# cs4247/music-transcription

Hardware: AMD Instinct MI355X
Metric: 30 s audio chunks/sec (mel+CNNRNN forward) (higher is better)
Workload: dtype f16; 1 GPU; CNNRNNModel inference, batch=32x30 s synthetic 16 kHz audio, mel+CNN-RNN HIP path (BASELINE.json configs[1]); batch_per_gpu=32, frames=938, coscheduled_batches_per_forward=4, streams_per_gpu=4, batches_in_flight=16, parallelism=dp1 (independent chunks)

## Files before the change

### music-transcription_amd/csrc/lstm.hip

```cpp
#include "lstm_handoff.h"
#include <stdlib.h>

namespace mt {

struct LstmArgs {
    const float* gx;
    const float* w_hh;
    float* hx;
    unsigned* status;
    int B, T, H;
    int g0;
    int ngl;
    float* gates_out;
    float* cx;
    const float* w_ihx;
    const float* bias;
    const float* hx_prev;
    int sleep_first, sleep_retry;
};

__device__ __forceinline__ float sigmoidf_(float x) { return __builtin_amdgcn_rcpf(1.0f + __expf(-x)); }
__device__ __forceinline__ float tanhf_(float x) { return fmaf(2.0f, __builtin_amdgcn_rcpf(1.0f + __expf(-2.0f * x)), -1.0f); }
constexpr unsigned H_POISON = 0xFFFFFFFFu;
constexpr int PAYLOAD_POLL_SLEEP = 10;
constexpr int PAYLOAD_POLL_SLEEP_BUSY = 18;
constexpr int PAYLOAD_POLL_SLEEP_TRAIN = 12;

#ifdef MT_LSTM_DIAG
__device__ unsigned long long mt_lstm_diag[1024][8];
#define DIAG_STAMP(i) do { if (tid == 0) { const long long n_ = __builtin_amdgcn_s_memrealtime(); dg[i] += n_ - tl; tl = n_; } } while (0)
#else
#define DIAG_STAMP(i) do { } while (0)
#endif

typedef __attribute__((__vector_size__(4 * sizeof(int)))) int i32x4_t;
__device__ __forceinline__ i32x4_t raw_rsrc(const void* p, unsigned bytes) {
    const unsigned long long a = (unsigned long long)p;
    i32x4_t r;
    r[0] = __builtin_amdgcn_readfirstlane((int)(unsigned)a);
    r[1] = __builtin_amdgcn_readfirstlane((int)((unsigned)(a >> 32) & 0xffffu));
    r[2] = __builtin_amdgcn_readfirstlane((int)bytes);
    r[3] = 0x00020000;
    return r;
}
__device__ __forceinline__ void asm_load_b128_sc1(u32x4& dst, int voff, i32x4_t rsrc) {
    asm volatile("buffer_load_dwordx4 %0, %1, %2, 0 offen sc1" : "=v"(dst) : "v"(voff), "s"(rsrc));
}
template <int N> __device__ __forceinline__ void vm_wait() { asm volatile("s_waitcnt vmcnt(%0)" :: "n"(N)); }
__device__ __forceinline__ void vm_settle(u32x4& v) { asm volatile("" : "+v"(v)); }

template <int NKSW, bool TRAIN = false, bool XP = false, int NG = 1, bool G16 = false>
__global__ __launch_bounds__(XP ? 256 : 320, XP ? 1 : (NKSW > 8 ? 2 : 4)) void lstm_rec_kernel(LstmArgs a) {
    __shared__ __attribute__((aligned(16))) float red[4][64][20];
    __shared__ __attribute__((aligned(16))) f16_t hs[32][8];
    constexpr int GX_RING = XP ? 1 : 6;
    constexpr int GX_DMA = G16 ? 2 : 4;
    __shared__ __attribute__((aligned(16))) float gring[GX_RING][XP ? 4 : (G16 ? 512 : 1024)];
    __shared__ int abort_s;
    const int tid = threadIdx.x, wv = tid >> 6, lane = tid & 63;
    const int H = a.H, T = a.T, nkb = H >> 3, nks = H >> 4;
    const int kb = blockIdx.x, d = blockIdx.y, gbase = blockIdx.z * NG + a.g0;
    const int ngh = min(NG, a.g0 + a.ngl - gbase);
    const int b = lane & 31, hh = lane >> 5;

    if (!XP && wv == 4) {
        typedef __attribute__((address_space(1))) void gvoid_t;
        typedef __attribute__((address_space(3))) void lvoid_t;
        const size_t gd_blocks_l = (size_t)T * 2 * nkb;
        const int nslots = T * ngh;
        int is = 0, ig = 0;
        auto request = [&](int n) {
            const int tn = d ? (T - 1 - is) : is;
            const size_t blk = (size_t)(gbase + ig) * gd_blocks_l + ((size_t)tn * 2 + d) * nkb + kb;
            const char* src = (const char*)a.gx + blk * (G16 ? 2048 : 4096) + lane * 16;
            char* dst = (char*)&gring[n % GX_RING][0];
#pragma unroll
            for (int qq = 0; qq < GX_DMA; ++qq) __builtin_amdgcn_global_load_lds((gvoid_t*)(src + qq * 1024), (lvoid_t*)(dst + qq * 1024), 16, 0, 0);
            if (++ig == ngh) { ig = 0; ++is; }
        };
        for (int n = 0; n < GX_RING - 1 && n < nslots; ++n) request(n);
        if (GX_RING - 1 <= nslots) asm volatile("s_waitcnt vmcnt(%0)" :: "n"(GX_DMA * (GX_RING - 2)) : "memory");
        else asm volatile("s_waitcnt vmcnt(0)" ::: "memory");
        __builtin_amdgcn_s_barrier();
        for (int n = 0; n < nslots; ++n) {
            if (n + GX_RING - 1 < nslots) {
                request(n + GX_RING - 1);
                asm volatile("s_waitcnt vmcnt(%0)" :: "n"(GX_DMA * (GX_RING - 2)) : "memory");
            } else {
                asm volatile("s_waitcnt vmcnt(0)" ::: "memory");
            }
            __builtin_amdgcn_s_barrier();
            int ab;
            asm volatile("ds_read_b32 %0, %1\n\ts_waitcnt lgkmcnt(0)" : "=v"(ab) : "v"((unsigned)(size_t)(lvoid_t*)&abort_s) : "memory");
            if (ab) return;
            __builtin_amdgcn_s_barrier();
        }
        return;
    }

    const int r = lane & 31, q = r >> 3, rh = (r >> 2) & 1, p = r & 3;
    const int wrow = p * H + kb * 8 + 2 * q + rh;
    const float* wsrc = a.w_hh + ((size_t)d * 4 * H + wrow) * H;
    f16x8 w16[NKSW];
#pragma unroll
    for (int i = 0; i < NKSW; ++i) {
        const int ks = wv * NKSW + i, ksc = min(ks, nks - 1);
        const f32x4 w0 = *(const f32x4*)(wsrc + ksc * 16 + 8 * hh), w1 = *(const f32x4*)(wsrc + ksc * 16 + 8 * hh + 4);
#pragma unroll
        for (int j = 0; j < 4; ++j) {
            w16[i][j] = (ks < nks) ? (f16_t)w0[j] : (f16_t)0.0f;
            w16[i][4 + j] = (ks < nks) ? (f16_t)w1[j] : (f16_t)0.0f;
        }
    }

    constexpr int NKSX = XP ? 2 * NKSW : 1;
    f16x8 wx[NKSX];
    if (XP) {
        const float* wxsrc = a.w_ihx + ((size_t)d * 4 * H + wrow) * (2 * H);
#pragma unroll
        for (int i = 0; i < NKSX; ++i) {
            const int kx = wv * NKSX + i, kxc = min(kx, 2 * nks - 1);
            const f32x4 w0 = *(const f32x4*)(wxsrc + kxc * 16 + 8 * hh), w1 = *(const f32x4*)(wxsrc + kxc * 16 + 8 * hh + 4);
#pragma unroll
            for (int j = 0; j < 4; ++j) {
                wx[i][j] = (kx < 2 * nks) ? (f16_t)w0[j] : (f16_t)0.0f;
                wx[i][4 + j] = (kx < 2 * nks) ? (f16_t)w1[j] : (f16_t)0.0f;
            }
        }
    }

    const int jl = 2 * wv + hh;
    float cst[NG];
#pragma unroll
    for (int gi = 0; gi < NG; ++gi) cst[gi] = 0.0f;
    float bias4[4] = {0.0f, 0.0f, 0.0f, 0.0f};
    if (XP) {
#pragma unroll
        for (int pp = 0; pp < 4; ++pp) bias4[pp] = a.bias[(size_t)d * 4 * H + pp * H + kb * 8 + jl];
    }
    const size_t gd_blocks = (size_t)T * 2 * nkb;
    if (tid == 0) abort_s = 0;
    __syncthreads();
#ifdef MT_LSTM_DIAG
    unsigned long long dg[8] = {0, 0, 0, 0, 0, 0, 0, 0};
    long long tl = __builtin_amdgcn_s_memrealtime();
#endif

    u32x4 hq[NKSW];
    const bool pf = NG > 1 && ngh > 1;
    int ring = 0;
    for (int s = 0; s < T; ++s) {
        const int t = d ? (T - 1 - s) : s;
        const int tprev = d ? (t + 1) : (t - 1);
#pragma unroll
      for (int gi = 0; gi < NG; ++gi) {
        if (gi >= ngh) continue;
        const int g = gbase + gi;
        const int Bg = min(32, a.B - g * 32);
        float& c = cst[gi];
        char* hx_g = (char*)a.hx + (size_t)g * gd_blocks * 512;
        const __amdgpu_buffer_rsrc_t hrsrc = __builtin_amdgcn_make_buffer_rsrc(hx_g, 0, (int)(gd_blocks * 512), 0x00020000);
        const __amdgpu_buffer_rsrc_t xrsrc = __builtin_amdgcn_make_buffer_rsrc(
            XP ? (void*)((const char*)a.hx_prev + (size_t)g * gd_blocks * 512) : (void*)hx_g, 0, (int)(gd_blocks * 512), 0x00020000);

        u32x4 xr[NKSX];
        if (XP) {
#pragma unroll
            for (int i = 0; i < NKSX; ++i) {
                const int kx = wv * NKSX + i, dsel = kx >= nks ? 1 : 0, ksx = kx - dsel * nks;
                xr[i] = __builtin_amdgcn_raw_buffer_load_b128(xrsrc, (kx < 2 * nks) ? ((t * 2 + dsel) * nkb) * 512 + ksx * 1024 + lane * 16 : OOB_OFF, 0, 0);
            }
        }
        float gxv[4];
        if (XP) {
#pragma unroll
            for (int pp = 0; pp < 4; ++pp) gxv[pp] = bias4[pp];
        } else if (G16) {
            unsigned short raw[4];
#pragma unroll
            for (int pp = 0; pp < 4; ++pp) raw[pp] = ((const unsigned short*)gring[ring])[pp * 256 + jl * 32 + b];
            __builtin_amdgcn_sched_barrier(0);
#pragma unroll
            for (int pp = 0; pp < 4; ++pp) gxv[pp] = (float)__builtin_bit_cast(f16_t, raw[pp]);
        } else {
#pragma unroll
            for (int pp = 0; pp < 4; ++pp) gxv[pp] = gring[ring][pp * 256 + jl * 32 + b];
        }
        ring = ring + 1 == GX_RING ? 0 : ring + 1;
        f32x16 acc, accx;
#pragma unroll
        for (int e = 0; e < 16; ++e) acc[e] = accx[e] = 0.0f;
        if (XP && s == 0) {
#pragma unroll
            for (int i = 0; i < NKSX; ++i) accx = __builtin_amdgcn_mfma_f32_32x32x16_f16(wx[i], __builtin_bit_cast(f16x8, xr[i]), accx, 0, 0, 0);
            acc = accx;
        }
        if (s > 0) {
            {
                if (NG == 1) sleep64(a.sleep_first);
            }
            const int hbase = ((tprev * 2 + d) * nkb) * 512 + lane * 16;
            long long t1 = 0;
            const i32x4_t hr = raw_rsrc(hx_g, (unsigned)(gd_blocks * 512));
            for (unsigned it = 0;; ++it) {
                if (!pf || it > 0) {
#pragma unroll
                    for (int i = 0; i < NKSW; ++i) {
                        const int ks = wv * NKSW + i;
                        if (NG > 1) asm_load_b128_sc1(hq[i], (ks < nks) ? hbase + ks * 1024 : OOB_OFF, hr);
                        else hq[i] = __builtin_amdgcn_raw_buffer_load_b128(hrsrc, (ks < nks) ? hbase + ks * 1024 : OOB_OFF, 0, 16 );
                    }
                }
                if (NG > 1) {
                    static_assert(NG == 1 || (!TRAIN && !XP), "NG > 1 is the plain inference kernel: the hand-counted vmcnt does not cover TRAIN / XP stores and loads");
                    if (pf && it == 0 && wv == 0) vm_wait<1>();
                    else vm_wait<0>();
#pragma unroll
                    for (int i = 0; i < NKSW; ++i) vm_settle(hq[i]);
                }
                if (XP) {
                    if (it == 0) {
                        __builtin_amdgcn_sched_barrier(0);
#pragma unroll
                        for (int i = 0; i < NKSX; ++i) accx = __builtin_amdgcn_mfma_f32_32x32x16_f16(wx[i], __builtin_bit_cast(f16x8, xr[i]), accx, 0, 0, 0);
                        __builtin_amdgcn_sched_barrier(0);
                    }
                    acc = accx;
                }
                unsigned worst = 0;
#pragma unroll
                for (int i = 0; i < NKSW; ++i) {
                    worst = max(max(worst, max(hq[i][0], hq[i][1])), max(hq[i][2], hq[i][3]));
                    acc = __builtin_amdgcn_mfma_f32_32x32x16_f16(w16[i], __builtin_bit_cast(f16x8, hq[i]), acc, 0, 0, 0);
                }
                if (!__any(worst == H_POISON)) break;
#ifdef MT_LSTM_DIAG
                if (tid == 0) dg[7] += 1;
#endif
#pragma unroll
                for (int e = 0; e < 16; ++e) acc[e] = 0.0f;
                sleep64(a.sleep_retry);
                if ((it & 63u) == 63u && __hip_atomic_load(a.status, __ATOMIC_RELAXED, __HIP_MEMORY_SCOPE_AGENT) != 0) {
                    if (lane == 0) abort_s = 1;
                    break;
                }
                if ((it & 255u) == 255u) {
                    const long long now = __builtin_amdgcn_s_memrealtime();
                    if (t1 == 0) t1 = now;
                    else if (now - t1 > LSTM_SPIN_LIMIT_TICKS) {
                        if (lane == 0) {
                            __hip_atomic_store(a.status, 0x40000000u + (unsigned)s, __ATOMIC_RELAXED, __HIP_MEMORY_SCOPE_AGENT);
                            abort_s = 1;
                        }
                        break;
                    }
                }
            }
        }
        const bool wrap = gi + 1 >= ngh;
        const int sn = s + (wrap ? 1 : 0), gn = wrap ? gbase : g + 1;
        if (pf) {
            if (sn > 0 && sn < T) {
                const int tpn = d ? (T - sn) : (sn - 1);
                const i32x4_t nr = raw_rsrc((char*)a.hx + (size_t)gn * gd_blocks * 512, (unsigned)(gd_blocks * 512));
                const int nbase = ((tpn * 2 + d) * nkb) * 512 + lane * 16;
#pragma unroll
                for (int i = 0; i < NKSW; ++i) {
                    const int ks = wv * NKSW + i;
                    asm_load_b128_sc1(hq[i], (ks < nks) ? nbase + ks * 1024 : OOB_OFF, nr);
                }
            }
        }
#ifdef MT_LSTM_DIAG
        asm volatile("" :: "v"(acc[0]));
#endif
        DIAG_STAMP(2);
#pragma unroll
        for (int e4 = 0; e4 < 4; ++e4)
            *(f32x4*)(&red[wv][lane][4 * e4]) = f32x4{acc[4 * e4], acc[4 * e4 + 1], acc[4 * e4 + 2], acc[4 * e4 + 3]};
        __syncthreads();
        DIAG_STAMP(3);
        if (abort_s) {
            if (NG > 1) vm_wait<0>();
            return;
        }
        float pre[4];
        {
            const f32x4 r0 = *(const f32x4*)(&red[0][lane][4 * wv]), r1 = *(const f32x4*)(&red[1][lane][4 * wv]);
            const f32x4 r2 = *(const f32x4*)(&red[2][lane][4 * wv]), r3 = *(const f32x4*)(&red[3][lane][4 * wv]);
#pragma unroll
            for (int pp = 0; pp < 4; ++pp)
                pre[pp] = ((r0[pp] + r1[pp]) + (r2[pp] + r3[pp])) + ((XP || b < Bg) ? gxv[pp] : 0.0f);
        }
        const float ig = sigmoidf_(pre[0]), fg = sigmoidf_(pre[1]), gg = tanhf_(pre[2]), og = sigmoidf_(pre[3]);
        c = fmaf(fg, c, ig * gg);
        const float hval = og * tanhf_(c);
        if (TRAIN && b < Bg) {
            float* go = a.gates_out + (size_t)g * gd_blocks * 1024 + (((size_t)t * 2 + d) * nkb + kb) * 1024 + jl * 32 + b;
            go[0] = ig; go[256] = fg; go[512] = gg; go[768] = og;
            a.cx[(size_t)g * gd_blocks * 256 + (((size_t)t * 2 + d) * nkb + kb) * 256 + jl * 32 + b] = c;
        }
#ifdef MT_LSTM_DIAG
        asm volatile("" :: "v"(hval));
#endif
        DIAG_STAMP(4);
        hs[b][jl] = (f16_t)hval;
        DIAG_STAMP(5);
        __syncthreads();
        if (wv == 0) {
            const u32x4 piece = *(const u32x4*)(&hs[b][0]);
            const int hoff = ((t * 2 + d) * nkb) * 512 + (kb >> 1) * 1024 + ((kb & 1) * 32 + b) * 16;
            __builtin_amdgcn_raw_buffer_store_b128(piece, hrsrc, lane < 32 ? hoff : OOB_OFF, 0, 16 );
        }
        DIAG_STAMP(6);
      }
    }
    if (NG > 1) vm_wait<0>();
#ifdef MT_LSTM_DIAG
    if (tid == 0) {
        const int wg = (blockIdx.z * gridDim.y + blockIdx.y) * gridDim.x + blockIdx.x;
        for (int i = 0; i < 8; ++i) mt_lstm_diag[wg & 1023][i] = dg[i];
    }
#endif
}

template <int NK, bool TRAIN, bool G16>
__global__ __launch_bounds__(320, 4) void lstm_rec16_kernel(LstmArgs a) {
    __shared__ __attribute__((aligned(16))) float red[4][2][64][4];
    __shared__ __attribute__((aligned(16))) f16_t hs[32][8];
    constexpr int GX_RING = 6;
    constexpr int GX_DMA = G16 ? 2 : 4;
    __shared__ __attribute__((aligned(16))) float gring[GX_RING][G16 ? 512 : 1024];
    __shared__ int abort_s;
    const int tid = threadIdx.x, wv = tid >> 6, lane = tid & 63;
    const int H = a.H, T = a.T, nkb = H >> 3, nks = H >> 4;
    const int kb = blockIdx.x, d = blockIdx.y, g = blockIdx.z + a.g0;
    const int Bg = min(16, a.B - g * 32);
    const size_t gd_blocks = (size_t)T * 2 * nkb;

    if (wv == 4) {
        typedef __attribute__((address_space(1))) void gvoid_t;
        typedef __attribute__((address_space(3))) void lvoid_t;
        int is = 0;
        auto request = [&](int n) {
            const int tn = d ? (T - 1 - is) : is;
            const size_t blk = (size_t)g * gd_blocks + ((size_t)tn * 2 + d) * nkb + kb;
            const char* src = (const char*)a.gx + blk * (G16 ? 2048 : 4096) + lane * 16;
            char* dst = (char*)&gring[n % GX_RING][0];
#pragma unroll
            for (int qq = 0; qq < GX_DMA; ++qq) __builtin_amdgcn_global_load_lds((gvoid_t*)(src + qq * 1024), (lvoid_t*)(dst + qq * 1024), 16, 0, 0);
            ++is;
        };
        for (int n = 0; n < GX_RING - 1 && n < T; ++n) request(n);
        if (GX_RING - 1 <= T) asm volatile("s_waitcnt vmcnt(%0)" :: "n"(GX_DMA * (GX_RING - 2)) : "memory");
        else asm volatile("s_waitcnt vmcnt(0)" ::: "memory");
        __builtin_amdgcn_s_barrier();
        for (int n = 0; n < T; ++n) {
            if (n + GX_RING - 1 < T) {
                request(n + GX_RING - 1);
                asm volatile("s_waitcnt vmcnt(%0)" :: "n"(GX_DMA * (GX_RING - 2)) : "memory");
            } else {
                asm volatile("s_waitcnt vmcnt(0)" ::: "memory");
            }
            __builtin_amdgcn_s_barrier();
            int ab;
            asm volatile("ds_read_b32 %0, %1\n\ts_waitcnt lgkmcnt(0)" : "=v"(ab) : "v"((unsigned)(size_t)(lvoid_t*)&abort_s) : "memory");
            if (ab) return;
            __builtin_amdgcn_s_barrier();
        }
        return;
    }

    const int rr = lane & 15, kg = lane >> 4;
    f16x8 w16[2][NK];
#pragma unroll
    for (int mt = 0; mt < 2; ++mt) {
        const int wrow = (rr & 3) * H + kb * 8 + 4 * mt + (rr >> 2);
        const float* wsrc = a.w_hh + ((size_t)d * 4 * H + wrow) * H;
#pragma unroll
        for (int i = 0; i < NK; ++i) {
            const int k0 = (wv * NK + i) * 32 + 8 * kg, k0c = min(k0, H - 8);
            const f32x4 w0 = *(const f32x4*)(wsrc + k0c), w1 = *(const f32x4*)(wsrc + k0c + 4);
#pragma unroll
            for (int j = 0; j < 4; ++j) {
                w16[mt][i][j] = (k0 < H) ? (f16_t)w0[j] : (f16_t)0.0f;
                w16[mt][i][4 + j] = (k0 < H) ? (f16_t)w1[j] : (f16_t)0.0f;
            }
        }
    }
    const int n = lane & 15, rg = lane >> 4, jl = 4 * (wv & 1) + rg;
    const bool owner = wv < 2;
    float c = 0.0f;
    char* hx_g = (char*)a.hx + (size_t)g * gd_blocks * 512;
    const __amdgpu_buffer_rsrc_t hrsrc = __builtin_amdgcn_make_buffer_rsrc(hx_g, 0, (int)(gd_blocks * 512), 0x00020000);
    const __amdgpu_buffer_rsrc_t gors = __builtin_amdgcn_make_buffer_rsrc(TRAIN ? (void*)(a.gates_out + (size_t)g * gd_blocks * 1024) : (void*)a.hx, 0,
                                                                          (int)(gd_blocks * 4096), 0x00020000);
    const __amdgpu_buffer_rsrc_t cxrs = __builtin_amdgcn_make_buffer_rsrc(TRAIN ? (void*)(a.cx + (size_t)g * gd_blocks * 256) : (void*)a.hx, 0,
                                                                          (int)(gd_blocks * 1024), 0x00020000);
    const int vo_t = (n < Bg) ? (jl * 32 + n) * 4 : 0x7FFFF000;
    if (tid == 0) abort_s = 0;
    if (tid < 128) ((unsigned*)&hs[0][0])[tid] = 0u;
    __syncthreads();

    int ring = 0;
    for (int s = 0; s < T; ++s) {
        const int t = d ? (T - 1 - s) : s;
        const int tprev = d ? (t + 1) : (t - 1);
        float gxv[4];
        if (G16) {
            unsigned short raw[4];
#pragma unroll
            for (int pp = 0; pp < 4; ++pp) raw[pp] = ((const unsigned short*)gring[ring])[pp * 256 + jl * 32 + n];
            __builtin_amdgcn_sched_barrier(0);
#pragma unroll
            for (int pp = 0; pp < 4; ++pp) gxv[pp] = (float)__builtin_bit_cast(f16_t, raw[pp]);
        } else {
#pragma unroll
            for (int pp = 0; pp < 4; ++pp) gxv[pp] = gring[ring][pp * 256 + jl * 32 + n];
        }
        ring = ring + 1 == GX_RING ? 0 : ring + 1;
        f32x4 acc[2] = {{0.0f, 0.0f, 0.0f, 0.0f}, {0.0f, 0.0f, 0.0f, 0.0f}};
        if (s > 0) {
            sleep64(a.sleep_first);
            const int hbase = ((tprev * 2 + d) * nkb) * 512 + ((kg & 1) * 32 + n) * 16 + (kg >> 1) * 1024;
            long long t1 = 0;
            for (unsigned it = 0;; ++it) {
                u32x4 hq[NK];
#pragma unroll
                for (int i = 0; i < NK; ++i) {
                    const int ks = 2 * (wv * NK + i) + (kg >> 1);
                    hq[i] = __builtin_amdgcn_raw_buffer_load_b128(hrsrc, (ks < nks) ? hbase + (wv * NK + i) * 2048 : OOB_OFF, 0, 16 );
                }
                unsigned worst = 0;
#pragma unroll
                for (int i = 0; i < NK; ++i) {
                    worst = max(max(worst, max(hq[i][0], hq[i][1])), max(hq[i][2], hq[i][3]));
                    acc[0] = __builtin_amdgcn_mfma_f32_16x16x32_f16(w16[0][i], __builtin_bit_cast(f16x8, hq[i]), acc[0], 0, 0, 0);
                    acc[1] = __builtin_amdgcn_mfma_f32_16x16x32_f16(w16[1][i], __builtin_bit_cast(f16x8, hq[i]), acc[1], 0, 0, 0);
                }
                if (!__any(worst == H_POISON)) break;
                acc[0] = f32x4{0.0f, 0.0f, 0.0f, 0.0f}; acc[1] = f32x4{0.0f, 0.0f, 0.0f, 0.0f};
                sleep64(a.sleep_retry);
                if ((it & 63u) == 63u && __hip_atomic_load(a.status, __ATOMIC_RELAXED, __HIP_MEMORY_SCOPE_AGENT) != 0) {
                    if (lane == 0) abort_s = 1;
                    break;
                }
                if ((it & 255u) == 255u) {
                    const long long now = __builtin_amdgcn_s_memrealtime();
                    if (t1 == 0) t1 = now;
                    else if (now - t1 > LSTM_SPIN_LIMIT_TICKS) {
                        if (lane == 0) {
                            __hip_atomic_store(a.status, 0x40000000u + (unsigned)s, __ATOMIC_RELAXED, __HIP_MEMORY_SCOPE_AGENT);
                            abort_s = 1;
                        }
                        break;
                    }
                }
            }
        }
        *(f32x4*)(&red[wv][0][lane][0]) = acc[0];
        *(f32x4*)(&red[wv][1][lane][0]) = acc[1];
        __syncthreads();
        if (abort_s) return;
        float gate[4] = {0.0f, 0.0f, 0.0f, 0.0f};
        if (owner) {
            const int mt = wv;
            const f32x4 r0 = *(const f32x4*)(&red[0][mt][lane][0]), r1 = *(const f32x4*)(&red[1][mt][lane][0]);
            const f32x4 r2 = *(const f32x4*)(&red[2][mt][lane][0]), r3 = *(const f32x4*)(&red[3][mt][lane][0]);
            float pre[4];
#pragma unroll
            for (int pp = 0; pp < 4; ++pp) pre[pp] = ((r0[pp] + r1[pp]) + (r2[pp] + r3[pp])) + (n < Bg ? gxv[pp] : 0.0f);
            gate[0] = sigmoidf_(pre[0]); gate[1] = sigmoidf_(pre[1]); gate[2] = tanhf_(pre[2]); gate[3] = sigmoidf_(pre[3]);
            c = fmaf(gate[1], c, gate[0] * gate[2]);
            hs[n][jl] = (f16_t)(gate[3] * tanhf_(c));
        }
        __syncthreads();
        if (wv == 0) {
            const u32x4 piece = *(const u32x4*)(&hs[lane & 31][0]);
            const int hoff = ((t * 2 + d) * nkb) * 512 + (kb >> 1) * 1024 + ((kb & 1) * 32 + (lane & 31)) * 16;
            __builtin_amdgcn_raw_buffer_store_b128(piece, hrsrc, lane < 32 ? hoff : OOB_OFF, 0, 16 );
        }
        if (TRAIN && owner) {
            const int so = __builtin_amdgcn_readfirstlane((t * 2 + d) * nkb + kb);
#pragma unroll
            for (int pp = 0; pp < 4; ++pp) __builtin_amdgcn_raw_buffer_store_b32(__builtin_bit_cast(unsigned, gate[pp]), gors, vo_t + pp * 1024, so * 4096, 0);
            __builtin_amdgcn_raw_buffer_store_b32(__builtin_bit_cast(unsigned, c), cxrs, vo_t, so * 1024, 0);
        }
    }
}

template <int DT>
__global__ void lstm_relayout_kernel(const f16_t* __restrict__ hx, bf16_t* __restrict__ X, int ldx, float* __restrict__ Y, int ldy,
                                     int col_off, int B, int T, int H, int Hv, Div3 dv, unsigned mB, unsigned sB) {
    const int nkb = H >> 3, nkv = (Hv + 7) >> 3;
    const unsigned total = (unsigned)T * B * 2 * nkv;
    for (unsigned id = blockIdx.x * blockDim.x + threadIdx.x; id < total; id += gridDim.x * blockDim.x) {
        int kb, d, mi;
        div3(id, dv, kb, d, mi);
        const size_t m = (size_t)mi;
        const int t = (int)fast_div((unsigned)mi, (unsigned)B, mB, sB), b = mi - t * B, g = b >> 5, bl = b & 31;
        const f16_t* src = hx + ((((size_t)g * T + t) * 2 + d) * nkb) * 256 + (size_t)(kb >> 1) * 512 + ((kb & 1) * 32 + bl) * 8;
        const int c0 = col_off + d * Hv + kb * 8;
        const f16x8 h8 = *(const f16x8*)src;
        if (X) {
            if (DT == MT_DT_F16 && (c0 & 7) == 0 && kb * 8 + 8 <= Hv) {
                *(f16x8*)(X + m * ldx + c0) = h8;
            } else if ((c0 & 7) == 0 && kb * 8 + 8 <= Hv) {
                *(uint4*)(X + m * ldx + c0) = make_uint4(pack_bf16x2((float)h8[0], (float)h8[1]), pack_bf16x2((float)h8[2], (float)h8[3]),
                                                         pack_bf16x2((float)h8[4], (float)h8[5]), pack_bf16x2((float)h8[6], (float)h8[7]));
            } else {
                for (int j = 0; j < 8 && kb * 8 + j < Hv; ++j) X[m * ldx + c0 + j] = f32_to_h16<DT>((float)h8[j]);
            }
        }
        if (Y)
            for (int j = 0; j < 8 && kb * 8 + j < Hv; ++j) Y[m * ldy + c0 + j] = (float)h8[j];
    }
}

__global__ void lstm_unpack_kernel(const f16_t* __restrict__ hx, float* __restrict__ y, int B, int T, int H) {
    const int nkb = H >> 3;
    const size_t total = (size_t)T * B * 2 * H;
    for (size_t id = (size_t)blockIdx.x * blockDim.x + threadIdx.x; id < total; id += (size_t)gridDim.x * blockDim.x) {
        const int k = id % H;
        const int d = (id / H) & 1;
        const size_t bt = id / (2 * H);
        const int t = bt % T, b = bt / T, g = b >> 5, bl = b & 31;
        const f16_t* blk = hx + ((((size_t)g * T + t) * 2 + d) * nkb) * 256 + (size_t)(k >> 4) * 512;
        y[id] = (float)blk[(((k >> 3) & 1) * 32 + bl) * 8 + (k & 7)];
    }
}

template <int NKSW, bool G16>
static int launch_rec_plain(const LstmArgs& a, int ngroups, hipStream_t st) {
    const dim3 one_set(a.H >> 3, 2, 1);
    if constexpr (NKSW <= 8) {
        if (ngroups == 2) return persistent_launch(lstm_rec_kernel<NKSW, false, false, 2, G16>, one_set, 320, a, st, "mt_lstm_bidir_fwd");
        if (ngroups == 3) return persistent_launch(lstm_rec_kernel<NKSW, false, false, 3, G16>, one_set, 320, a, st, "mt_lstm_bidir_fwd");
        if (ngroups > 3) return persistent_launch(lstm_rec_kernel<NKSW, false, false, 4, G16>, dim3(a.H >> 3, 2, cdiv(ngroups, 4)), 320, a, st, "mt_lstm_bidir_fwd");
    }
    return persistent_launch(lstm_rec_kernel<NKSW, false, false, 1, G16>, dim3(a.H >> 3, 2, ngroups), 320, a, st, "mt_lstm_bidir_fwd");
}

template <int NKSW>
static int launch_rec(const LstmArgs& a, int ngroups, bool g16, hipStream_t st) {
    const dim3 per_group(a.H >> 3, 2, ngroups);
    if constexpr (NKSW <= 8) {
        static const bool c16 = !(getenv("MT_LSTM_C16") && atoi(getenv("MT_LSTM_C16")) == 0);
        constexpr int NK16 = (NKSW + 1) / 2;
        if (c16 && !a.w_ihx && a.B <= 16 && ngroups == 1) {
            if (a.cx) return persistent_launch(lstm_rec16_kernel<NK16, true, false>, per_group, 320, a, st, "mt_lstm_bidir_fwd_train");
            if (g16) return persistent_launch(lstm_rec16_kernel<NK16, false, true>, per_group, 320, a, st, "mt_lstm_bidir_fwd");
            return persistent_launch(lstm_rec16_kernel<NK16, false, false>, per_group, 320, a, st, "mt_lstm_bidir_fwd");
        }
        if (a.w_ihx) return persistent_launch(lstm_rec_kernel<NKSW, false, true>, per_group, 256, a, st, "mt_lstm_bidir_fwd_xproj");
    }
    if (a.cx) return persistent_launch(lstm_rec_kernel<NKSW, true, false>, per_group, 320, a, st, "mt_lstm_bidir_fwd_train");
    return g16 ? launch_rec_plain<NKSW, true>(a, ngroups, st) : launch_rec_plain<NKSW, false>(a, ngroups, st);
}

}

using namespace mt;

extern "C" size_t mt_lstm_gx_bytes(int B, int T, int H) { return (size_t)cdiv(B, 32) * T * 2 * (H >> 3) * 4096; }
extern "C" size_t mt_lstm_hx_bytes(int B, int T, int H) { return (size_t)cdiv(B, 32) * T * 2 * (H >> 3) * 512; }
extern "C" size_t mt_lstm_sync_bytes(int B, int H) { (void)B; (void)H; return 512; }

static int lstm_fwd_impl(const float* gx, const float* w_hh, float* hx, void* sync_ws, size_t sync_bytes,
                         int B, int T, int H, int flags, mt_stream_t stream, float* cx = nullptr,
                         const float* w_ihx = nullptr, const float* bias = nullptr, const float* hx_prev = nullptr) {
    MT_REQUIRE((gx || w_ihx) && w_hh && hx && sync_ws, MT_EINVAL, "mt_lstm_bidir_fwd: null pointer");
    MT_REQUIRE(B > 0 && T > 0 && H >= 16 && H % 16 == 0 && H <= 1024, MT_EUNSUPPORTED,
               "mt_lstm_bidir_fwd: hidden size %d unsupported (multiple of 16, <= 1024)", H);
    MT_REQUIRE(sync_bytes >= mt_lstm_sync_bytes(B, H), MT_EWORKSPACE, "mt_lstm_bidir_fwd: sync workspace too small");
    const int nkb = H >> 3, ng = cdiv(B, 32);
    const bool g16 = (flags & MT_GX_F16) != 0;
    MT_REQUIRE(!g16 || (!cx && !w_ihx), MT_EINVAL, "mt_lstm_bidir_fwd_ex: MT_GX_F16 is for plain inference launches only");
    MT_REQUIRE((size_t)T * 2 * nkb * 512 < ((size_t)1 << 31), MT_EUNSUPPORTED, "mt_lstm_bidir_fwd: T*H too large for one buffer descriptor");
    MT_REQUIRE(!cx || (size_t)T * 2 * nkb * 4096 < ((size_t)1 << 31), MT_EUNSUPPORTED, "mt_lstm_bidir_fwd_train: T*H too large for one buffer descriptor of the gates");
    MT_REQUIRE((((size_t)w_hh | (size_t)w_ihx) & 15) == 0, MT_EINVAL, "mt_lstm_bidir_fwd: weight matrices must be 16-byte aligned");
    hipStream_t st = (hipStream_t)stream;
    MT_CHECK_HIP(hipMemsetAsync(sync_ws, 0, mt_lstm_sync_bytes(B, H), st));
    MT_CHECK_HIP(hipMemsetAsync(hx, 0xFF, mt_lstm_hx_bytes(B, T, H), st));
    static const int env_first = getenv("MT_LSTM_POLL_FIRST") ? atoi(getenv("MT_LSTM_POLL_FIRST")) : -1;
    static const int env_retry = getenv("MT_LSTM_POLL_RETRY") ? atoi(getenv("MT_LSTM_POLL_RETRY")) : -1;
    LstmArgs a{gx, w_hh, hx, (unsigned*)sync_ws, B, T, H, 0, 0,
               cx ? const_cast<float*>(gx) : nullptr, cx, w_ihx, bias, hx_prev,
               env_first >= 0 ? env_first : (cx ? PAYLOAD_POLL_SLEEP_TRAIN : ((!w_ihx && mt_persistent_cus_in_flight(stream) > 0) ? PAYLOAD_POLL_SLEEP_BUSY : PAYLOAD_POLL_SLEEP)),
               env_retry >= 0 ? env_retry : 0};
    const int zmax = (256 / (2 * nkb)) > 0 ? (256 / (2 * nkb)) : 1;
    const int nksw = cdiv(nkb / 2, 4);
    const int per_launch = (cx || w_ihx || nksw > 8) ? zmax : 4 * zmax;
    for (int g0 = 0; g0 < ng; g0 += per_launch) {
        a.g0 = g0;
        const int n = (ng - g0) < per_launch ? (ng - g0) : per_launch;
        a.ngl = n;
        int rc;
        if (nksw <= 1) rc = launch_rec<1>(a, n, g16, st);
        else if (nksw <= 2) rc = launch_rec<2>(a, n, g16, st);
        else if (nksw <= 4) rc = launch_rec<4>(a, n, g16, st);
        else if (nksw <= 8) rc = launch_rec<8>(a, n, g16, st);
        else rc = launch_rec<16>(a, n, g16, st);
        if (rc != MT_OK) return rc;
    }
    return MT_OK;
}

extern "C" int mt_lstm_bidir_fwd(const float* gx, const float* w_hh, float* hx, void* sync_ws, size_t sync_bytes,
                                 int B, int T, int H, mt_stream_t stream) {
    return lstm_fwd_impl(gx, w_hh, hx, sync_ws, sync_bytes, B, T, H, 0, stream);
}

extern "C" int mt_lstm_bidir_fwd_xproj(const float* hx_prev, const float* w_ihx, const float* bias, const float* w_hh, float* hx,
                                       void* sync_ws, size_t sync_bytes, int B, int T, int H, mt_stream_t stream) {
    MT_REQUIRE(hx_prev && w_ihx && bias && hx_prev != hx, MT_EINVAL, "mt_lstm_bidir_fwd_xproj: bad arguments");
    MT_REQUIRE(H <= 512, MT_EUNSUPPORTED, "mt_lstm_bidir_fwd_xproj: H=%d > 512 (the W_ih slice lives in registers)", H);
    return lstm_fwd_impl(nullptr, w_hh, hx, sync_ws, sync_bytes, B, T, H, 0, stream, nullptr, w_ihx, bias, hx_prev);
}

extern "C" int mt_lstm_bidir_fwd_train(float* gx_inout, const float* w_hh, float* hx, float* cx, void* sync_ws, size_t sync_bytes,
                                       int B, int T, int H, mt_stream_t stream) {
    MT_REQUIRE(cx, MT_EINVAL, "mt_lstm_bidir_fwd_train: null cx");
    return lstm_fwd_impl(gx_inout, w_hh, hx, sync_ws, sync_bytes, B, T, H, 0, stream, cx);
}

extern "C" int mt_lstm_bidir_fwd_ex(const float* gx, const float* w_hh, float* hx, void* sync_ws, size_t sync_bytes,
                                    int B, int T, int H, int flags, mt_stream_t stream) {
    MT_REQUIRE(flags == 0 || flags == MT_GX_F16, MT_EINVAL, "mt_lstm_bidir_fwd_ex: flags must be 0 or MT_GX_F16 (gx is f16)");
    return lstm_fwd_impl(gx, w_hh, hx, sync_ws, sync_bytes, B, T, H, flags, stream);
}

extern "C" int mt_lstm_relayout_dt(const float* hx, void* X, int ldx, float* Y, int ldy, int col_off, int B, int T, int H, int Hv,
                                   int dt, mt_stream_t stream) {
    MT_REQUIRE(hx && (X || Y) && H % 16 == 0 && Hv > 0 && Hv <= H && col_off >= 0, MT_EINVAL, "mt_lstm_relayout_ex: bad arguments");
    MT_REQUIRE((!X || (ldx >= col_off + 2 * Hv && ldx % 8 == 0)) && (!Y || ldy >= col_off + 2 * Hv), MT_EINVAL, "mt_lstm_relayout_ex: bad leading dimension");
    MT_REQUIRE_DT(dt, "mt_lstm_relayout");
    const size_t total = (size_t)T * B * 2 * ((Hv + 7) >> 3);
    MT_REQUIRE(total < ((size_t)1 << 31), MT_EUNSUPPORTED, "mt_lstm_relayout: more than 2^31 pieces");
    const int blocks = (int)((total + 255) / 256 < 4096 ? (total + 255) / 256 : 4096);
    const Div3 dv = make_div3((Hv + 7) >> 3, 2);
    unsigned mB, sB;
    div_magic((unsigned)B, &mB, &sB);
    if (dt == MT_DT_F16)
        hipLaunchKernelGGL(lstm_relayout_kernel<MT_DT_F16>, dim3(blocks), dim3(256), 0, (hipStream_t)stream, (const f16_t*)hx, (bf16_t*)X, ldx, Y, ldy,
                           col_off, B, T, H, Hv, dv, mB, sB);
    else
        hipLaunchKernelGGL(lstm_relayout_kernel<MT_DT_BF16>, dim3(blocks), dim3(256), 0, (hipStream_t)stream, (const f16_t*)hx, (bf16_t*)X, ldx, Y, ldy,
                           col_off, B, T, H, Hv, dv, mB, sB);
    MT_CHECK_LAUNCH();
    return MT_OK;
}
extern "C" int mt_lstm_relayout_ex(const float* hx, void* X, int ldx, float* Y, int ldy, int col_off, int B, int T, int H, int Hv,
                                   mt_stream_t stream) {
    return mt_lstm_relayout_dt(hx, X, ldx, Y, ldy, col_off, B, T, H, Hv, MT_DT_BF16, stream);
}

extern "C" int mt_lstm_relayout_bf16(const float* hx, void* X, int ldx, int B, int T, int H, mt_stream_t stream) {
    return mt_lstm_relayout_ex(hx, X, ldx, nullptr, 0, 0, B, T, H, H, stream);
}

#ifdef MT_LSTM_DIAG
extern "C" int mt_lstm_diag_read(unsigned long long* host_out ) {
    MT_CHECK_HIP(hipMemcpyFromSymbol(host_out, HIP_SYMBOL(mt_lstm_diag), sizeof(unsigned long long) * 1024 * 8));
    return MT_OK;
}
#endif

extern "C" int mt_lstm_unpack_f32(const float* hx, float* y, int B, int T, int H, mt_stream_t stream) {
    MT_REQUIRE(hx && y, MT_EINVAL, "mt_lstm_unpack_f32: null pointer");
    const size_t total = (size_t)T * B * 2 * H;
    const int blocks = (int)((total + 255) / 256 < 4096 ? (total + 255) / 256 : 4096);
    hipLaunchKernelGGL(lstm_unpack_kernel, dim3(blocks), dim3(256), 0, (hipStream_t)stream, (const f16_t*)hx, y, B, T, H);
    MT_CHECK_LAUNCH();
    return MT_OK;
}
```

Before: 8420 chunks/s.

## Trim LSTM recurrent spin-loop address math and register pressure

```diff
diff --git a/music-transcription_amd/csrc/lstm.hip b/music-transcription_amd/csrc/lstm.hip
--- a/music-transcription_amd/csrc/lstm.hip
+++ b/music-transcription_amd/csrc/lstm.hip
@@ -43,8 +43,17 @@
     r[3] = 0x00020000;
     return r;
 }
-__device__ __forceinline__ void asm_load_b128_sc1(u32x4& dst, int voff, i32x4_t rsrc) {
-    asm volatile("buffer_load_dwordx4 %0, %1, %2, 0 offen sc1" : "=v"(dst) : "v"(voff), "s"(rsrc));
+template <int OFF> __device__ __forceinline__ void asm_load_b128_sc1(u32x4& dst, int voff, i32x4_t rsrc) {
+    asm volatile("buffer_load_dwordx4 %0, %1, %2, 0 offen offset:%3 sc1" : "=v"(dst) : "v"(voff), "s"(rsrc), "n"(OFF));
+}
+template <int NKSW, int I = 0> __device__ __forceinline__ void asm_gather_sc1(u32x4 (&hq)[NKSW], int voff, i32x4_t rsrc) {
+    if constexpr (I < NKSW) {
+        asm_load_b128_sc1<(I & 3) * 1024>(hq[I], voff + (I >> 2) * 4096, rsrc);
+        asm_gather_sc1<NKSW, I + 1>(hq, voff, rsrc);
+    }
+}
+__device__ __forceinline__ unsigned spin_clock() {
+    return (unsigned)__builtin_amdgcn_readfirstlane((int)(unsigned)__builtin_amdgcn_s_memrealtime()) | 1u;
 }
 template <int N> __device__ __forceinline__ void vm_wait() { asm volatile("s_waitcnt vmcnt(%0)" :: "n"(N)); }
 __device__ __forceinline__ void vm_settle(u32x4& v) { asm volatile("" : "+v"(v)); }
@@ -57,7 +66,7 @@
     constexpr int GX_DMA = G16 ? 2 : 4;
     __shared__ __attribute__((aligned(16))) float gring[GX_RING][XP ? 4 : (G16 ? 512 : 1024)];
     __shared__ int abort_s;
-    const int tid = threadIdx.x, wv = tid >> 6, lane = tid & 63;
+    const int tid = threadIdx.x, wv = __builtin_amdgcn_readfirstlane(tid >> 6), lane = tid & 63;
     const int H = a.H, T = a.T, nkb = H >> 3, nks = H >> 4;
     const int kb = blockIdx.x, d = blockIdx.y, gbase = blockIdx.z * NG + a.g0;
     const int ngh = min(NG, a.g0 + a.ngl - gbase);
@@ -132,7 +141,10 @@
     const int jl = 2 * wv + hh;
     float cst[NG];
 #pragma unroll
-    for (int gi = 0; gi < NG; ++gi) cst[gi] = 0.0f;
+    for (int gi = 0; gi < NG; ++gi) {
+        cst[gi] = 0.0f;
+        if (NG > 1) red[wv][lane][16 + gi] = 0.0f;
+    }
     float bias4[4] = {0.0f, 0.0f, 0.0f, 0.0f};
     if (XP) {
 #pragma unroll
@@ -148,6 +160,8 @@
 
     u32x4 hq[NKSW];
     const bool pf = NG > 1 && ngh > 1;
+    int gvoff = wv * (NKSW * 1024) + lane * 16;
+    asm volatile("" : "+v"(gvoff));
     int ring = 0;
     for (int s = 0; s < T; ++s) {
         const int t = d ? (T - 1 - s) : s;
@@ -157,7 +171,7 @@
         if (gi >= ngh) continue;
         const int g = gbase + gi;
         const int Bg = min(32, a.B - g * 32);
-        float& c = cst[gi];
+        float& c = cst[NG > 1 ? 0 : gi];
         char* hx_g = (char*)a.hx + (size_t)g * gd_blocks * 512;
         const __amdgpu_buffer_rsrc_t hrsrc = __builtin_amdgcn_make_buffer_rsrc(hx_g, 0, (int)(gd_blocks * 512), 0x00020000);
         const __amdgpu_buffer_rsrc_t xrsrc = __builtin_amdgcn_make_buffer_rsrc(
@@ -172,16 +186,11 @@
             }
         }
         float gxv[4];
+        const int ring_cur = ring;
         if (XP) {
 #pragma unroll
             for (int pp = 0; pp < 4; ++pp) gxv[pp] = bias4[pp];
         } else if (G16) {
-            unsigned short raw[4];
-#pragma unroll
-            for (int pp = 0; pp < 4; ++pp) raw[pp] = ((const unsigned short*)gring[ring])[pp * 256 + jl * 32 + b];
-            __builtin_amdgcn_sched_barrier(0);
-#pragma unroll
-            for (int pp = 0; pp < 4; ++pp) gxv[pp] = (float)__builtin_bit_cast(f16_t, raw[pp]);
         } else {
 #pragma unroll
             for (int pp = 0; pp < 4; ++pp) gxv[pp] = gring[ring][pp * 256 + jl * 32 + b];
@@ -199,16 +208,17 @@
             {
                 if (NG == 1) sleep64(a.sleep_first);
             }
-            const int hbase = ((tprev * 2 + d) * nkb) * 512 + lane * 16;
-            long long t1 = 0;
-            const i32x4_t hr = raw_rsrc(hx_g, (unsigned)(gd_blocks * 512));
+            const char* himg = hx_g + (size_t)((tprev * 2 + d) * nkb) * 512;
+            unsigned t1 = 0;
+            int gave_up = 0;
+            const i32x4_t hr = raw_rsrc(himg, (unsigned)(nkb * 512));
+            const __amdgpu_buffer_rsrc_t hr1 = __builtin_amdgcn_make_buffer_rsrc((void*)himg, 0, nkb * 512, 0x00020000);
             for (unsigned it = 0;; ++it) {
                 if (!pf || it > 0) {
-#pragma unroll
-                    for (int i = 0; i < NKSW; ++i) {
-                        const int ks = wv * NKSW + i;
-                        if (NG > 1) asm_load_b128_sc1(hq[i], (ks < nks) ? hbase + ks * 1024 : OOB_OFF, hr);
-                        else hq[i] = __builtin_amdgcn_raw_buffer_load_b128(hrsrc, (ks < nks) ? hbase + ks * 1024 : OOB_OFF, 0, 16 );
+                    if constexpr (NG > 1) asm_gather_sc1<NKSW>(hq, gvoff, hr);
+                    else {
+#pragma unroll
+                        for (int i = 0; i < NKSW; ++i) hq[i] = __builtin_amdgcn_raw_buffer_load_b128(hr1, gvoff + i * 1024, 0, 16 );
                     }
                 }
                 if (NG > 1) {
@@ -240,21 +250,22 @@
 #pragma unroll
                 for (int e = 0; e < 16; ++e) acc[e] = 0.0f;
                 sleep64(a.sleep_retry);
-                if ((it & 63u) == 63u && __hip_atomic_load(a.status, __ATOMIC_RELAXED, __HIP_MEMORY_SCOPE_AGENT) != 0) {
-                    if (lane == 0) abort_s = 1;
+                if ((it & 63u) == 63u && __builtin_amdgcn_readfirstlane((int)__hip_atomic_load(a.status, __ATOMIC_RELAXED, __HIP_MEMORY_SCOPE_AGENT)) != 0) {
+                    gave_up = 1;
                     break;
                 }
                 if ((it & 255u) == 255u) {
-                    const long long now = __builtin_amdgcn_s_memrealtime();
+                    const unsigned now = spin_clock();
                     if (t1 == 0) t1 = now;
-                    else if (now - t1 > LSTM_SPIN_LIMIT_TICKS) {
-                        if (lane == 0) {
-                            __hip_atomic_store(a.status, 0x40000000u + (unsigned)s, __ATOMIC_RELAXED, __HIP_MEMORY_SCOPE_AGENT);
-                            abort_s = 1;
-                        }
+                    else if (now - t1 > (unsigned)LSTM_SPIN_LIMIT_TICKS) {
+                        gave_up = 2;
                         break;
                     }
                 }
+            }
+            if (gave_up && lane == 0) {
+                if (gave_up == 2) __hip_atomic_store(a.status, 0x40000000u + (unsigned)s, __ATOMIC_RELAXED, __HIP_MEMORY_SCOPE_AGENT);
+                abort_s = 1;
             }
         }
         const bool wrap = gi + 1 >= ngh;
@@ -262,13 +273,8 @@
         if (pf) {
             if (sn > 0 && sn < T) {
                 const int tpn = d ? (T - sn) : (sn - 1);
-                const i32x4_t nr = raw_rsrc((char*)a.hx + (size_t)gn * gd_blocks * 512, (unsigned)(gd_blocks * 512));
-                const int nbase = ((tpn * 2 + d) * nkb) * 512 + lane * 16;
-#pragma unroll
-                for (int i = 0; i < NKSW; ++i) {
-                    const int ks = wv * NKSW + i;
-                    asm_load_b128_sc1(hq[i], (ks < nks) ? nbase + ks * 1024 : OOB_OFF, nr);
-                }
+                const i32x4_t nr = raw_rsrc((char*)a.hx + ((size_t)gn * gd_blocks + (size_t)((tpn * 2 + d) * nkb)) * 512, (unsigned)(nkb * 512));
+                asm_gather_sc1<NKSW>(hq, gvoff, nr);
             }
         }
 #ifdef MT_LSTM_DIAG
@@ -286,6 +292,14 @@
         }
         float pre[4];
         {
+            if (G16 && !XP) {
+                unsigned short raw[4];
+#pragma unroll
+                for (int pp = 0; pp < 4; ++pp) raw[pp] = ((const unsigned short*)gring[ring_cur])[pp * 256 + jl * 32 + b];
+#pragma unroll
+                for (int pp = 0; pp < 4; ++pp) gxv[pp] = (float)__builtin_bit_cast(f16_t, raw[pp]);
+            }
+            if (NG > 1) c = red[wv][lane][16 + gi];
             const f32x4 r0 = *(const f32x4*)(&red[0][lane][4 * wv]), r1 = *(const f32x4*)(&red[1][lane][4 * wv]);
             const f32x4 r2 = *(const f32x4*)(&red[2][lane][4 * wv]), r3 = *(const f32x4*)(&red[3][lane][4 * wv]);
 #pragma unroll
@@ -295,6 +309,7 @@
         const float ig = sigmoidf_(pre[0]), fg = sigmoidf_(pre[1]), gg = tanhf_(pre[2]), og = sigmoidf_(pre[3]);
         c = fmaf(fg, c, ig * gg);
         const float hval = og * tanhf_(c);
+        if (NG > 1) red[wv][lane][16 + gi] = c;
         if (TRAIN && b < Bg) {
             float* go = a.gates_out + (size_t)g * gd_blocks * 1024 + (((size_t)t * 2 + d) * nkb + kb) * 1024 + jl * 32 + b;
             go[0] = ig; go[256] = fg; go[512] = gg; go[768] = og;
@@ -307,10 +322,10 @@
         hs[b][jl] = (f16_t)hval;
         DIAG_STAMP(5);
         __syncthreads();
-        if (wv == 0) {
+        if (wv == 0 && lane < 32) {
             const u32x4 piece = *(const u32x4*)(&hs[b][0]);
             const int hoff = ((t * 2 + d) * nkb) * 512 + (kb >> 1) * 1024 + ((kb & 1) * 32 + b) * 16;
-            __builtin_amdgcn_raw_buffer_store_b128(piece, hrsrc, lane < 32 ? hoff : OOB_OFF, 0, 16 );
+            __builtin_amdgcn_raw_buffer_store_b128(piece, hrsrc, hoff, 0, 16 );
         }
         DIAG_STAMP(6);
       }
```

After: 8830 chunks/s, median of 6. 4.9% higher.
